# wuliwei9278/primalCR

Measured on NVIDIA B200. Metric: sec_per_outer_iter_primalcrpp_k100_netflix_shape, lower is better.
Workload: dtype f64

## Files before the change

primalcr_b200/csrc/common.cuh:

```cuda
#pragma once
#include <cuda_runtime.h>
#include <stdint.h>
#include <stdio.h>
#include <stdlib.h>
#include <string>
#include <vector>
#include <map>
#include <stdexcept>

namespace pcr {

typedef long long i64;

struct Error : public std::runtime_error {
    int code;
    Error(int c, const std::string &w) : std::runtime_error(w), code(c) {}
};

#define PCR_CUDA(call)                                                                         \
    do {                                                                                       \
        cudaError_t _e = (call);                                                               \
        if (_e != cudaSuccess) {                                                               \
            char _b[512];                                                                      \
            snprintf(_b, sizeof(_b), "CUDA error %s at %s:%d: %s", cudaGetErrorName(_e),       \
// ... 48 lines not shown
                if (tf) {
                    float t0 = 0;
                    cudaEventElapsedTime(&t0, pending.front().a, r.a);
                    fprintf(tf, "%.4f %.4f %s\n", t0, ms, acc[r.id].name.c_str());
                }
            }
            pool.push_back(r.a); pool.push_back(r.b);
        }
        pending.clear();
        if (tf) { fprintf(tf, "# batch end\n"); fclose(tf); }
    }
    void reset() { resolve(); for (auto &a : acc) { a.ms = 0; a.launches = 0; a.bytes = 0; } }
    ~Profiler() { for (auto &r : pending) { cudaEventDestroy(r.a); cudaEventDestroy(r.b); } for (auto e : pool) cudaEventDestroy(e); }
};

struct DevPool {
    std::vector<void *> ptrs;
    i64 bytes = 0;
    cudaStream_t stream = nullptr;
    bool async = false;
    void init(cudaStream_t s) {
        stream = s;
        int dev = 0; cudaMemPool_t mp;
        if (cudaGetDevice(&dev) != cudaSuccess || cudaDeviceGetDefaultMemPool(&mp, dev) != cudaSuccess) { cudaGetLastError(); return; }
        async = true;
        unsigned long long keep = ~0ull;
        cudaMemPoolSetAttribute(mp, cudaMemPoolAttrReleaseThreshold, &keep);
    }
    void *raw_alloc(size_t b) {
        void *p = nullptr;
        if (b == 0) b = 1;
        if (async) PCR_CUDA(cudaMallocAsync(&p, b, stream)); else PCR_CUDA(cudaMalloc(&p, b));
        return p;
    }
    void raw_free(void *p) {
        if (!p) return;
        if (async) cudaFreeAsync(p, stream); else cudaFree(p);
    }
    template <typename T> T *alloc(size_t n) {
        const size_t b = (n > 0 ? n : 1) * sizeof(T);
        void *p = raw_alloc(b);
        ptrs.push_back(p); bytes += (i64)b;
        return (T *)p;
    }
    void release() {
        for (void *p : ptrs) raw_free(p);
        if (async && stream && !ptrs.empty()) cudaStreamSynchronize(stream);
        ptrs.clear(); bytes = 0;
    }
    ~DevPool() { release(); }
};

struct TileList { int32_t *first = nullptr, *nusers = nullptr, *ne = nullptr; i64 *e0 = nullptr; i64 n = 0, nnz = 0; };

struct DevCsr {
    i64 d1 = 0, nnz = 0;
    i64 *row_ptr = nullptr;
    int32_t *item = nullptr;
    int32_t *user = nullptr;
    double *rating = nullptr;
    uint8_t *level = nullptr;
    std::vector<i64> h_row_ptr;
    int32_t *cls_users[3] = {nullptr, nullptr, nullptr};
    int n_cls[3] = {0, 0, 0};
    i64 *heavy_off = nullptr;
    i64 heavy_total = 0;
    i64 *heavy_begin = nullptr, *heavy_end = nullptr;
    i64 max_len = 0;
    TileList tiles[3];
    int32_t *pt_user = nullptr; int32_t *pt_j0 = nullptr; i64 n_pt = 0;
    i64 *pt_ptr = nullptr;
    int32_t *un_seg = nullptr; i64 *un_start = nullptr; i64 n_units = 0;
    i64 *seg_unit_ptr = nullptr;
};

struct SortedMeta {
    double *s = nullptr;
    int32_t *pos = nullptr;
    uint8_t *lev = nullptr;
    int32_t *ub = nullptr, *lb = nullptr;
    int32_t *cnt_lo = nullptr, *cnt_hi = nullptr;
    double *lm_s = nullptr;
    unsigned long long *lm_w0 = nullptr, *lm_w1 = nullptr, *lm_w2 = nullptr;
    uint16_t *ulev = nullptr;
    i64 nnz = 0;
};

static const int HEAVY_CHUNK = 2048;
struct HeavyLM {
    int n_users = 0, n_chunks = 0;
    const int32_t *users = nullptr;
    const i64 *begin = nullptr, *end = nullptr;
    const i64 *off = nullptr;
    const int32_t *chunk_user = nullptr;
    const int32_t *chunk_lo = nullptr;
    const int32_t *chunk0 = nullptr;
    int32_t *ccnt = nullptr;
    int32_t *B = nullptr;
    int32_t *idx = nullptr;
    int32_t *pos = nullptr, *lo = nullptr, *hi = nullptr;
    uint8_t *lev = nullptr;
    double *G = nullptr, *G2 = nullptr;
    double *csum = nullptr;
    i64 htot = 0;
};

struct HeavySortPlan {
    int n_users = 0, n_chunks = 0, max_passes = 0;
    const i64 *begin = nullptr, *end = nullptr;
    const i64 *off = nullptr;
    const int32_t *chunk_user = nullptr;
    const int32_t *chunk_lo = nullptr;
    double *tmp_s = nullptr; int32_t *tmp_pos = nullptr;
};

static const int TILE_CAP = 1024;
static const int TILE_MAX_USERS = 128;
static const int TILE_CAP_M = 2048;
static const int TILE_CAP_L = 4096;
static const int S_CAP = 1024;
static const int L_CAP = 4096;
#ifndef PCR_ROWSUM_CHUNK
#define PCR_ROWSUM_CHUNK 256
#endif
static const int ROWSUM_CHUNK = PCR_ROWSUM_CHUNK;
static const int PAIR_TJ = 256;
static const int MAX_LEVELS = 256;

}
```

primalcr_b200/csrc/engine.cu:

```cuda
#include "kernels.h"
#include "../../include/primalcr.h"
#include "../host/loader.hpp"
#include "../host/textio.hpp"

#include <algorithm>
#include <chrono>
#include <cmath>
#include <cstring>
#include <dlfcn.h>
#include <random>
#include <mutex>

typedef struct { char internal[128]; } pcr_ncclUniqueId;
typedef void *pcr_ncclComm_t;
enum { PCR_NCCL_FLOAT64 = 8, PCR_NCCL_SUM = 0 };

namespace pcr {

struct NcclApi {
    void *h = nullptr;
    int (*GetUniqueId)(pcr_ncclUniqueId *) = nullptr;
    int (*CommInitRank)(pcr_ncclComm_t *, int, pcr_ncclUniqueId, int) = nullptr;
    int (*AllReduce)(const void *, void *, size_t, int, int, pcr_ncclComm_t, cudaStream_t) = nullptr;
    int (*ReduceScatter)(const void *, void *, size_t, int, int, pcr_ncclComm_t, cudaStream_t) = nullptr;
// ... 310 lines not shown
                c0.push_back((int32_t)cu.size());
                for (i64 lo = 0; lo < he[q] - hb[q]; lo += HEAVY_CHUNK) { cu.push_back((int32_t)q); clo.push_back((int32_t)lo); }
            }
            c0.push_back((int32_t)cu.size());
            hv.n_users = (int)cls[2].size(); hv.n_chunks = (int)cu.size(); hv.htot = htot;
            hv.users = X.cls_users[2]; hv.begin = X.heavy_begin; hv.end = X.heavy_end;
            hv.off = upload_vec(hoff_h); hv.chunk_user = upload_vec(cu); hv.chunk_lo = upload_vec(clo); hv.chunk0 = upload_vec(c0);
            hv.ccnt = pool.alloc<int32_t>((size_t)hv.n_chunks * 8); hv.B = pool.alloc<int32_t>((size_t)hv.n_users * 9);
            hv.idx = pool.alloc<int32_t>((size_t)std::max(T - 1, 1) * (size_t)htot);
            hv.G = pool.alloc<double>((size_t)htot); hv.G2 = pool.alloc<double>((size_t)htot);
            hv.pos = pool.alloc<int32_t>((size_t)htot); hv.lo = pool.alloc<int32_t>((size_t)htot); hv.hi = pool.alloc<int32_t>((size_t)htot);
            hv.lev = pool.alloc<uint8_t>((size_t)htot);
            hv.csum = pool.alloc<double>((size_t)hv.n_chunks * 2);
            sync();
        } else {
            alloc_heavy_cta_scratch();
        }
        {
            std::vector<int32_t> useg; std::vector<i64> ustart, supt;
            make_units(X.h_row_ptr, useg, ustart, supt);
            X.n_units = (i64)useg.size();
            X.un_seg = upload_vec(useg); X.un_start = upload_vec(ustart); X.seg_unit_ptr = upload_vec(supt);
            sync();
        }
        lap("classes, tiles, user units");
        col_ptr = pool.alloc<i64>((size_t)d2 + 1);
        csc2csr = pool.alloc<int32_t>((size_t)nnz); csc_user = pool.alloc<int32_t>((size_t)nnz);
        k_build_csc(ctx, pool, X.item, X.user, nnz, d2, col_ptr, csc2csr, csc_user);
        std::vector<i64> h_col((size_t)d2 + 1);
        PCR_CUDA(cudaMemcpyAsync(h_col.data(), col_ptr, sizeof(i64) * ((size_t)d2 + 1), cudaMemcpyDeviceToHost, stream));
        sync();
        PCR_REQUIRE(h_col[d2] == nnz, "item id out of range [0, d2)");
        lap("CSC build (device)");
        {
            const double blk_bytes = getenv("PRIMALCR_UBLOCK_MB") ? atof(getenv("PRIMALCR_UBLOCK_MB")) * 1e6 : 24e6;
            const double u_bytes = (double)d1 * ld * 8.0;
            int nb = (int)std::ceil(u_bytes / blk_bytes);
            if (getenv("PRIMALCR_UBLOCK_MB") == nullptr) {
                const i64 nb_max = std::max<i64>(1, nnz / (32 * std::max<i64>(d2, 1)));
                if (nb > nb_max) nb = (int)nb_max;
            }
            if (nb < 1) nb = 1;
            if (nb > 64) nb = 64;
            const i64 bu = (d1 + nb - 1) / nb > 0 ? (d1 + nb - 1) / nb : 1;
            n_user_blocks = nb;
            std::vector<i64> bpos((size_t)d2 * (nb + 1));
            i64 *bpos_d = nullptr;
            bpos_d = (i64 *)pool.raw_alloc(sizeof(i64) * bpos.size());
            k_csc_block_bounds(ctx, col_ptr, csc_user, d2, nb, bu, bpos_d);
            PCR_CUDA(cudaMemcpyAsync(bpos.data(), bpos_d, sizeof(i64) * bpos.size(), cudaMemcpyDeviceToHost, stream));
            sync();
            pool.raw_free(bpos_d);
            std::vector<int32_t> cseg, cidx; std::vector<i64> cstart, cend, csup((size_t)d2 + 1, 0);
            for (int blk = 0; blk < nb; ++blk)
                for (i64 pcol = 0; pcol < d2; ++pcol) {
                    const i64 lo = bpos[(size_t)pcol * (nb + 1) + blk], hi = blk + 1 == nb ? h_col[pcol + 1] : bpos[(size_t)pcol * (nb + 1) + blk + 1];
                    const i64 collen = h_col[pcol + 1] - h_col[pcol];
                    const i64 chunk = std::max<i64>(ROWSUM_CHUNK, (collen + 47) / 48);
                    for (i64 bb = lo; bb < hi; bb += chunk) {
                        cseg.push_back((int32_t)pcol); cstart.push_back(bb); cend.push_back(std::min(bb + chunk, hi));
                        csup[pcol + 1] += 1;
                    }
                }
            n_cunits = (i64)cseg.size();
            for (i64 pcol = 0; pcol < d2; ++pcol) csup[pcol + 1] += csup[pcol];
            cidx.resize(cseg.size());
            std::vector<i64> fill(csup.begin(), csup.end() - 1);
            for (size_t uu = 0; uu < cseg.size(); ++uu) cidx[fill[cseg[uu]]++] = (int32_t)uu;
            cu_seg = upload_vec(cseg); cu_start = upload_vec(cstart); cu_end = upload_vec(cend);
            col_unit_ptr = upload_vec(csup); col_unit_idx = upload_vec(cidx);
            sync();
        }
        lap("item units (user blocks)");
        m = pool.alloc<double>((size_t)nnz); b = pool.alloc<double>((size_t)nnz); cbuf = pool.alloc<double>((size_t)nnz);
        meta.s = pool.alloc<double>((size_t)nnz); meta.pos = pool.alloc<int32_t>((size_t)nnz);
        meta.lev = pool.alloc<uint8_t>((size_t)nnz);
        meta.ub = pool.alloc<int32_t>((size_t)nnz); meta.lb = pool.alloc<int32_t>((size_t)nnz);
        meta.cnt_lo = pool.alloc<int32_t>((size_t)nnz); meta.cnt_hi = pool.alloc<int32_t>((size_t)nnz);
        meta.nnz = nnz;
        if (use_tiles) {
            meta.lm_s = pool.alloc<double>((size_t)nnz);
            meta.lm_w0 = pool.alloc<unsigned long long>((size_t)nnz); meta.lm_w1 = pool.alloc<unsigned long long>((size_t)nnz);
            if (T > 5) meta.lm_w2 = pool.alloc<unsigned long long>((size_t)nnz);
            meta.ulev = pool.alloc<uint16_t>((size_t)d1 * 8);
            PCR_CUDA(cudaMemsetAsync(meta.ulev, 0, sizeof(uint16_t) * (size_t)d1 * 8, stream));
        }
        const size_t vn = (size_t)d2 * ld, un = (size_t)d1 * ld;
        U = pool.alloc<double>(un);
        d2p = world > 1 ? (d2 + world - 1) / world * world : d2;
        vs_rows = d2p / std::max(world, 1); vs_row0 = (i64)rank * vs_rows;
        sharded_cg = world > 1 && (double)vn * 8.0 >= 64e6;
        if (const char *sc_env = getenv("PRIMALCR_SHARDED_CG")) sharded_cg = world > 1 && atoi(sc_env) != 0;
        const size_t vnp = (size_t)d2p * ld;
        g = pool.alloc<double>(vnp); delta = pool.alloc<double>(vnp); rr = pool.alloc<double>(vnp);
        p = pool.alloc<double>(vnp); Hp = pool.alloc<double>(vnp); V = pool.alloc<double>(vnp); Vnew = pool.alloc<double>(vnp);
        for (double *vec : {g, delta, rr, p, Hp, V, Vnew}) PCR_CUDA(cudaMemsetAsync(vec, 0, sizeof(double) * vnp, stream));
        partial = pool.alloc<double>((size_t)std::max(X.n_units, n_cunits) * ld);
        us.g = pool.alloc<double>(un); us.delta = pool.alloc<double>(un); us.rr = pool.alloc<double>(un);
        us.p = pool.alloc<double>(un); us.Hp = pool.alloc<double>(un); us.Unew = pool.alloc<double>(un);
        us.err = pool.alloc<double>((size_t)d1); us.step = pool.alloc<double>((size_t)d1);
        us.prev_obj = pool.alloc<double>((size_t)d1); us.obj_new = pool.alloc<double>((size_t)d1);
        us.loss = pool.alloc<double>((size_t)d1);
        us.cg_active = pool.alloc<uint8_t>((size_t)d1); us.ls_active = pool.alloc<uint8_t>((size_t)d1);
        us.skipped = pool.alloc<uint8_t>((size_t)d1);
        us.cg_its = pool.alloc<int32_t>((size_t)d1); us.ls_trials = pool.alloc<int32_t>((size_t)d1);
        k_fill(ctx, us.loss, d1, 0.0);
        has_pairs = pool.alloc<uint8_t>((size_t)d1);
        k_has_pairs(ctx, X, has_pairs);
        obj_item = pool.alloc<double>((size_t)X.n_pt);
        ensure_eval_buffers(X);
        sync();
        lap("work buffers");
        has_train = true;
    }

    void alloc_heavy_cta_scratch() {
        if (h_v != nullptr || X.heavy_total <= 0) return;
        const size_t htot = (size_t)X.heavy_total;
        h_v = pool.alloc<double>(htot); h_p1 = pool.alloc<double>(htot);
        h_p2 = pool.alloc<double>(htot); h_acc = pool.alloc<double>(htot);
        h_cnt = pool.alloc<int32_t>(htot);
    }
    void ensure_heavy_windows() {
        if (!heavy_chunked || heavy_windows_valid || X.n_cls[2] == 0) return;
        alloc_heavy_cta_scratch();
        k_windows(ctx, 2, X.cls_users[2], X.n_cls[2], nullptr, X.row_ptr, meta, T, X.heavy_off, h_cnt);
        heavy_windows_valid = true;
    }
    i64 ev_cap_pt = 0, ev_cap_d1 = 0, ev_cap_nnz = 0;
    void ensure_eval_buffers(const DevCsr &C) {
        if (C.n_pt > ev_cap_pt) { ev_err_item = pool.alloc<i64>((size_t)C.n_pt); ev_cap_pt = C.n_pt; }
        if (C.d1 > ev_cap_d1 || ev_a == nullptr) {
            ev_err_user = pool.alloc<i64>((size_t)C.d1);
            ev_a = pool.alloc<double>((size_t)C.d1); ev_b = pool.alloc<double>((size_t)C.d1);
            ev_c = pool.alloc<double>((size_t)C.d1); ev_d = pool.alloc<double>((size_t)C.d1); ev_cap_d1 = C.d1;
        }
    }

    void set_test(i64 nnz, const i64 *row_ptr, const int32_t *item, const double *rating) {
        bind();
        PCR_REQUIRE(has_train, "load the training set first");
        PCR_REQUIRE(!has_test, "test set already loaded");
        build_csr_common(XT, d1, nnz, row_ptr, item, rating);
        ev_score_t = pool.alloc<double>((size_t)nnz);
        ensure_eval_buffers(XT);
        has_test = nnz > 0;
    }

    void put_matrix(const double *h, i64 rows, double *dst) {
        if (rows == 0) return;
        if (ld == k) {
            PCR_CUDA(cudaMemcpyAsync(dst, h, sizeof(double) * (size_t)rows * k, cudaMemcpyHostToDevice, stream));
        } else {
            double *tmp = (double *)pool.raw_alloc(sizeof(double) * (size_t)rows * k);
            PCR_CUDA(cudaMemcpyAsync(tmp, h, sizeof(double) * (size_t)rows * k, cudaMemcpyHostToDevice, stream));
            k_pad_copy(ctx, tmp, rows, k, ld, dst);
            PCR_CUDA(cudaStreamSynchronize(stream));
            pool.raw_free(tmp);
        }
    }
    void get_matrix(const double *src, i64 rows, double *h) {
        if (rows == 0) return;
        if (ld == k) {
            PCR_CUDA(cudaMemcpyAsync(h, src, sizeof(double) * (size_t)rows * k, cudaMemcpyDeviceToHost, stream));
        } else {
            PCR_CUDA(cudaMemcpy2DAsync(h, sizeof(double) * k, src, sizeof(double) * ld, sizeof(double) * k, (size_t)rows,
                                       cudaMemcpyDeviceToHost, stream));
        }
// ... 797 lines not shown
```

primalcr_b200/csrc/k_tiles.cu:

```cuda
#include "kernels.h"
#include <math_constants.h>

namespace pcr {

#define FULL 0xffffffffu
#define LAUNCH(ctx, name, bytes, kernel, grid, block, smem, ...)                         \
    do {                                                                                 \
        (ctx).prof->begin(name, (ctx).stream, (double)(bytes));                          \
        kernel<<<(grid), (block), (smem), (ctx).stream>>>(__VA_ARGS__);                  \
        (ctx).prof->end((ctx).stream);                                                   \
        PCR_CUDA(cudaGetLastError());                                                    \
    } while (0)

static const int TE = 4;

template <int CAP>
struct TileShared {
    int ustart[TILE_MAX_USERS + 1];
    uint8_t uact[TILE_MAX_USERS];
    uint8_t ul[CAP];
};

template <typename VT, int TT, int TH, typename ValF, typename LevF>
__device__ __forceinline__ void tile_level_scan(const TileShared<TH * TE> &ts, int ne, int T, VT *S, VT *wagg ,
                                                int *wflag , ValF val, LevF lev) {
    constexpr int SLOTS = TH * TE + TILE_MAX_USERS;
    const int tid = threadIdx.x, lane = tid & 31, warp = tid >> 5;
    const int lo = tid * TE;
    VT agg[TT];
#pragma unroll
    for (int t = 0; t < TT; ++t) agg[t] = (VT)0;
    int flag = 0;
#pragma unroll
    for (int q = 0; q < TE; ++q) {
        const int i = lo + q;
        if (i < ne) {
            const int u = ts.ul[i];
            if (i == ts.ustart[u]) {
#pragma unroll
                for (int t = 0; t < TT; ++t) agg[t] = (VT)0;
                flag = 1;
            }
            const int l = lev(i);
            const VT v = val(i);
#pragma unroll
            for (int t = 0; t < TT; ++t) agg[t] += (t == l) ? v : (VT)0;
        }
    }
    VT inc[TT];
#pragma unroll
    for (int t = 0; t < TT; ++t) inc[t] = agg[t];
    int finc = flag;
#pragma unroll
    for (int o = 1; o < 32; o <<= 1) {
        const int of = __shfl_up_sync(FULL, finc, o);
#pragma unroll
        for (int t = 0; t < TT; ++t) {
            const VT ov = __shfl_up_sync(FULL, inc[t], o);
            if (lane >= o && !finc) inc[t] += ov;
        }
        if (lane >= o) finc |= of;
    }
    if (lane == 31) {
#pragma unroll
        for (int t = 0; t < TT; ++t) wagg[warp * TT + t] = inc[t];
        wflag[warp] = finc;
    }
    VT exc[TT];
    int fexc = __shfl_up_sync(FULL, finc, 1);
#pragma unroll
    for (int t = 0; t < TT; ++t) { exc[t] = __shfl_up_sync(FULL, inc[t], 1); if (lane == 0) exc[t] = (VT)0; }
    if (lane == 0) fexc = 0;
    __syncthreads();
    VT carry[TT];
#pragma unroll
    for (int t = 0; t < TT; ++t) carry[t] = (VT)0;
    for (int w = 0; w < warp; ++w) {
        const int wf = wflag[w];
#pragma unroll
        for (int t = 0; t < TT; ++t) carry[t] = wf ? wagg[w * TT + t] : carry[t] + wagg[w * TT + t];
    }
#pragma unroll
    for (int t = 0; t < TT; ++t) carry[t] = fexc ? exc[t] : carry[t] + exc[t];
#pragma unroll
    for (int q = 0; q < TE; ++q) {
        const int i = lo + q;
        if (i < ne) {
            const int u = ts.ul[i];
            if (i == ts.ustart[u]) {
#pragma unroll
                for (int t = 0; t < TT; ++t) carry[t] = (VT)0;
            }
            const int slot = i + u;
#pragma unroll
            for (int t = 0; t < TT; ++t) if (t < T) S[t * SLOTS + slot] = carry[t];
            const int l = lev(i);
            const VT v = val(i);
#pragma unroll
            for (int t = 0; t < TT; ++t) carry[t] += (t == l) ? v : (VT)0;
            if (i + 1 == ts.ustart[u + 1]) {
#pragma unroll
                for (int t = 0; t < TT; ++t) if (t < T) S[t * SLOTS + slot + 1] = carry[t];
            }
        }
    }
    __syncthreads();
}

template <int TH>
__device__ __forceinline__ bool tile_users(TileShared<TH * TE> &ts, int first_user, int n_users, i64 e0,
                                           const i64 *__restrict__ row_ptr, const uint8_t *__restrict__ active) {
    const int tid = threadIdx.x;
    int any = 0;
    for (int u = tid; u <= n_users; u += TH) {
        const i64 rp = row_ptr[first_user + u];
        ts.ustart[u] = (int)(rp - e0);
        if (u < n_users) {
            const uint8_t a = active ? active[first_user + u] : (uint8_t)1;
            ts.uact[u] = a;
            if (a && row_ptr[first_user + u + 1] > rp) any = 1;
        }
    }
    return __syncthreads_or(any) != 0;
}

#ifndef PCR_PREP_MINB
#define PCR_PREP_MINB 4
#endif
template <int TT, int TH>
__global__ void __launch_bounds__(TH, TH == 256 ? PCR_PREP_MINB : (TH == 512 ? 2 : 1)) tile_prepare_kernel(const int32_t *__restrict__ tile_first,
                                                          const int32_t *__restrict__ tile_nusers,
                                                          const i64 *__restrict__ tile_e0, const int32_t *__restrict__ tile_ne,
                                                          const uint8_t *__restrict__ active,
                                                          const i64 *__restrict__ row_ptr, const int32_t *__restrict__ user_of,
                                                          const double *__restrict__ m, const uint8_t *__restrict__ level,
                                                          double *__restrict__ s_out, int32_t *__restrict__ pos_out,
                                                          uint8_t *__restrict__ lev_out, int32_t *__restrict__ ub_out,
                                                          int32_t *__restrict__ lb_out, int32_t *__restrict__ lo_out,
                                                          int32_t *__restrict__ hi_out, int T, SortedMeta lm) {
    constexpr int CAP = TH * TE, SLOTS = CAP + TILE_MAX_USERS;
    extern __shared__ __align__(16) unsigned char smraw[];
    __shared__ TileShared<CAP> ts;
    __shared__ int wagg[TH / 32 * TT];
    __shared__ int wflag[TH / 32];
    double *keys = reinterpret_cast<double *>(smraw);
    unsigned long long *pk = reinterpret_cast<unsigned long long *>(keys + CAP);
    int *C = reinterpret_cast<int *>(pk + CAP);
    uint32_t *tag = reinterpret_cast<uint32_t *>(C + T * SLOTS);
    uint8_t *slev = reinterpret_cast<uint8_t *>(tag + CAP);
    uint8_t *lev0 = slev + CAP;
    __shared__ int s_fallback;
    const int tid = threadIdx.x;
    const int first_user = tile_first[blockIdx.x], n_users = tile_nusers[blockIdx.x];
    const i64 e0 = tile_e0[blockIdx.x];
    const int ne = tile_ne[blockIdx.x];
    bool users_done = false;
    if (active) {
        if (!tile_users<TH>(ts, first_user, n_users, e0, row_ptr, active)) return;
        users_done = true;
    }
    int np2 = 1;
    while (np2 < ne) np2 <<= 1;
    double r_m[TE]; int r_u[TE]; uint8_t r_l[TE];
#pragma unroll
    for (int q = 0; q < TE; ++q) {
        const int i = tid + q * TH;
        r_m[q] = CUDART_INF; r_u[q] = 0xFFFF; r_l[q] = 0;
        if (i < ne) { r_m[q] = m[e0 + i]; r_u[q] = user_of[e0 + i] - first_user; r_l[q] = level[e0 + i]; }
    }
    if (!users_done) tile_users<TH>(ts, first_user, n_users, e0, row_ptr, active);
#pragma unroll
    for (int q = 0; q < TE; ++q) {
        const int i = tid + q * TH;
        if (i < np2) {
            keys[i] = r_m[q];
            if (i < ne) {
                const float f = (float)r_m[q] + 0.0f;
                const uint32_t b = __float_as_uint(f);
                const uint32_t fk = b ^ ((b >> 31) ? 0xFFFFFFFFu : 0x80000000u);
                pk[i] = ((unsigned long long)r_u[q] << 45) | ((unsigned long long)fk << 13) | (unsigned long long)i;
                ts.ul[i] = (uint8_t)r_u[q]; lev0[i] = r_l[q];
            } else {
                pk[i] = ~0ull;
            }
        }
    }
    if (tid == 0) s_fallback = 0;
    __syncthreads();
    {
        const int p0 = tid * TE;
        const bool live = ((tid & ~31) * TE) < np2;
        unsigned long long ek[TE];
#pragma unroll
        for (int q = 0; q < TE; ++q) ek[q] = pk[p0 + q];
        for (int k = 2; k <= np2; k <<= 1) {
            for (int j = k >> 1; j >= 32 * TE; j >>= 1) {
                __syncthreads();
#pragma unroll
                for (int q = 0; q < TE; ++q) pk[p0 + q] = ek[q];
                __syncthreads();
                const int m = j / TE;
                const int pp = (tid ^ m) * TE;
                const bool keep_min = (((tid & m) == 0) == ((p0 & k) == 0));
#pragma unroll
                for (int q = 0; q < TE; ++q) {
                    const unsigned long long o = pk[pp + q];
// ... 17 lines not shown
                    for (int q = 0; q < 2; ++q) {
                        const unsigned long long a = ek[q], b = ek[q + 2];
                        if ((a > b) == asc) { ek[q] = b; ek[q + 2] = a; }
                    }
                }
#pragma unroll
                for (int q = 0; q < TE; q += 2) {
                    const bool asc = (((p0 + q) & k) == 0);
                    const unsigned long long a = ek[q], b = ek[q + 1];
                    if ((a > b) == asc) { ek[q] = b; ek[q + 1] = a; }
                }
            }
        }
        __syncthreads();
#pragma unroll
        for (int q = 0; q < TE; ++q) pk[p0 + q] = ek[q];
        __syncthreads();
    }
    {
        int round = 0;
        for (;;) {
            int swapped = 0;
            for (int phase = 0; phase < 2; ++phase) {
                for (int i = 2 * tid + phase; i + 1 < ne; i += 2 * TH) {
                    const unsigned long long a = pk[i], b = pk[i + 1];
                    if ((a >> 13) == (b >> 13)) {
                        const int ia = (int)(a & 0x1FFFu), ib = (int)(b & 0x1FFFu);
                        const double ka = keys[ia], kb = keys[ib];
                        if (ka > kb || (ka == kb && ia > ib)) { pk[i] = b; pk[i + 1] = a; swapped = 1; }
                    }
                }
                __syncthreads();
            }
            if (!__syncthreads_or(swapped)) break;
            if (++round >= 48) { if (tid == 0) s_fallback = 1; break; }
        }
        __syncthreads();
    }
    const bool fallback = s_fallback != 0;
    double srt[TE];
#pragma unroll
    for (int q = 0; q < TE; ++q) {
        const int i = tid + q * TH;
        srt[q] = CUDART_INF;
        if (i < ne && !fallback) srt[q] = keys[(int)(pk[i] & 0x1FFFu)];
    }
    __syncthreads();
#pragma unroll
    for (int q = 0; q < TE; ++q) {
        const int i = tid + q * TH;
        if (i < np2) {
            if (!fallback) {
                if (i < ne) { keys[i] = srt[q]; tag[i] = ((uint32_t)ts.ul[i] << 16) | (uint32_t)(pk[i] & 0x1FFFu); }
            } else {
                keys[i] = r_m[q];
                tag[i] = i < ne ? (((uint32_t)r_u[q] << 16) | (uint32_t)i) : 0xFFFFFFFFu;
            }
        }
    }
    __syncthreads();
    if (fallback) {
        for (int k = 2; k <= np2; k <<= 1) {
            for (int j = k >> 1; j > 0; j >>= 1) {
                for (int t = tid; t < (np2 >> 1); t += TH) {
                    const int i = ((t & ~(j - 1)) << 1) | (t & (j - 1));
                    const int p = i | j;
                    const bool asc = (i & k) == 0;
                    const uint32_t ti = tag[i], tp = tag[p];
                    const double ki = keys[i], kp = keys[p];
                    const bool gt = ((ti >> 16) != (tp >> 16)) ? (ti > tp) : ((ki > kp) || (ki == kp && ti > tp));
                    if (gt == asc) { keys[i] = kp; keys[p] = ki; tag[i] = tp; tag[p] = ti; }
                }
                __syncthreads();
            }
        }
    }
    for (int i = tid; i < ne; i += TH) {
        const int src = (int)(tag[i] & 0xFFFFu);
        const uint8_t l = lev0[src];
        slev[i] = l;
        if (ts.uact[ts.ul[i]]) { s_out[e0 + i] = keys[i]; pos_out[e0 + i] = (int32_t)(e0 + src); lev_out[e0 + i] = l; }
    }
    __syncthreads();
    tile_level_scan<int, TT, TH>(ts, ne, T, C, wagg, wflag, [](int) { return 1; }, [&](int i) { return (int)slev[i]; });
    for (int i = tid; i < ne; i += TH) {
        const int u = ts.ul[i];
        if (!ts.uact[u]) continue;
        const int u0 = ts.ustart[u], n = ts.ustart[u + 1] - u0, x = i - u0;
        const double *kk = keys + u0;
        const double sj = kk[x];
        const double hi = __dadd_rn(sj, 1.0), lo = __dadd_rn(sj, -1.0);
        int a = x + 1, b = n;
        while (a < b) { const int mid = (a + b) >> 1; if (kk[mid] <= hi) a = mid + 1; else b = mid; }
        const int ub = a;
        a = 0; b = x;
        while (a < b) { const int mid = (a + b) >> 1; if (kk[mid] < lo) a = mid + 1; else b = mid; }
        const int lb = a;
        const int base = u0 + u, l = slev[i];
        int chi = 0, clo = 0;
        for (int t = 0; t < T; ++t) {
            const int *Ct = C + t * SLOTS + base;
            if (t > l) chi += Ct[ub];
            else if (t < l) clo += Ct[n] - Ct[lb];
        }
        ub_out[e0 + i] = ub; lb_out[e0 + i] = lb; lo_out[e0 + i] = clo; hi_out[e0 + i] = chi;
        int run = 0, r = 0;
        uint16_t other[TT];
#pragma unroll
        for (int t = 0; t < TT; ++t) {
            other[t] = 0;
            if (t < T) {
                const int *Ct = C + t * SLOTS + base;
                if (t == l) r = run + Ct[x];
                else other[t] = (uint16_t)(run + (t > l ? Ct[ub] : Ct[lb]));
                run += Ct[n];
            }
        }
        const i64 gi = e0 + u0 + r;
        unsigned long long w1 = 0ull, w2 = 0ull;
#pragma unroll
        for (int t = 0; t < TT; ++t) {
            if (t < T && t != l) {
                const int slot = t < l ? t : t - 1;
                if (slot < 4) w1 |= (unsigned long long)other[t] << (13 * slot);
                else          w2 |= (unsigned long long)other[t] << (13 * (slot - 4));
            }
        }
        lm.lm_s[gi] = sj;
        lm.lm_w0[gi] = (unsigned long long)(tag[i] & 0xFFFFu) | ((unsigned long long)clo << 13) | ((unsigned long long)chi << 26) |
                       ((unsigned long long)l << 39) | ((unsigned long long)u << 42);
        lm.lm_w1[gi] = w1;
        if (TT > 5) lm.lm_w2[gi] = w2;
    }
    for (int w = tid; w < n_users * T; w += TH) {
        const int u = w / T, t = w - u * T;
        const int n = ts.ustart[u + 1] - ts.ustart[u];
        if (ts.uact[u]) lm.ulev[(i64)(first_user + u) * 8 + t] = (uint16_t)(n > 0 ? C[t * SLOTS + ts.ustart[u] + u + n] : 0);
    }
}

#ifndef PCR_LM_MINB
#define PCR_LM_MINB 5
#endif
template <int MODE, int TT, int TH>
__global__ void __launch_bounds__(TH, TH == 256 ? PCR_LM_MINB : (TH == 512 ? 2 : 1)) tile_lm_sweep_kernel(const int32_t *__restrict__ tile_first,
                                                           const int32_t *__restrict__ tile_nusers,
                                                           const i64 *__restrict__ tile_e0, const int32_t *__restrict__ tile_ne,
                                                           const uint8_t *__restrict__ active,
                                                           const i64 *__restrict__ row_ptr, const int32_t *__restrict__ user_of,
                                                           SortedMeta lm, const double *__restrict__ b_g,
                                                           double *__restrict__ c_out, double *__restrict__ obj_user, int T) {
    constexpr int CAP = TH * TE, SLOTS = CAP + TILE_MAX_USERS;
    __shared__ TileShared<CAP> ts;
    __shared__ double wagg[TH / 32];
    __shared__ int wflag[TH / 32];
    extern __shared__ __align__(16) unsigned char smraw[];
    double *G = reinterpret_cast<double *>(smraw);
    double *sval = G + SLOTS;
    double *G2 = sval + CAP;
    double *stg = sval + CAP;
    __shared__ double Kt[TILE_MAX_USERS * TT], Kt2[MODE == 2 ? TILE_MAX_USERS * TT : 1];
    __shared__ uint16_t Bt[TILE_MAX_USERS * (TT + 1)];
    const int tid = threadIdx.x;
    const int first_user = tile_first[blockIdx.x], n_users = tile_nusers[blockIdx.x];
    const i64 e0 = tile_e0[blockIdx.x];
    const int ne = tile_ne[blockIdx.x];
    bool users_done = false;
    if (active) {
        if (!tile_users<TH>(ts, first_user, n_users, e0, row_ptr, active)) return;
        users_done = true;
    }
    unsigned long long r_w0[TE], r_w1[TE], r_w2[TT > 5 ? TE : 1];
    double r_v[TE];
#pragma unroll
    for (int q = 0; q < TE; ++q) {
        const int i = tid + q * TH;
        r_w0[q] = 0ull; r_w1[q] = 0ull; r_v[q] = 0.0;
        if (TT > 5) r_w2[q] = 0ull;
        if (i < ne) {
            r_w0[q] = lm.lm_w0[e0 + i];
            r_w1[q] = lm.lm_w1[e0 + i];
            if (TT > 5) r_w2[q] = lm.lm_w2[e0 + i];
            if (MODE != 1) r_v[q] = lm.lm_s[e0 + i];
        }
    }
    if (MODE == 1) {
#pragma unroll
        for (int q = 0; q < TE; ++q) { const int i = tid + q * TH; if (i < ne) stg[i] = b_g[e0 + i]; }
    }
    if (!users_done) tile_users<TH>(ts, first_user, n_users, e0, row_ptr, active);
    for (int u = tid; u < n_users; u += TH) {
        int run = 0;
        for (int t = 0; t < T; ++t) { Bt[u * (TT + 1) + t] = (uint16_t)run; run += lm.ulev[(i64)(first_user + u) * 8 + t]; }
        Bt[u * (TT + 1) + T] = (uint16_t)run;
    }
#pragma unroll
    for (int q = 0; q < TE; ++q) {
        const int i = tid + q * TH;
        if (i < ne) { ts.ul[i] = (uint8_t)((r_w0[q] >> 42) & 0x7Full); if (MODE != 1) sval[i] = MODE == 2 ? r_v[q] - 1.0 : r_v[q]; }
    }
    __syncthreads();
    if (MODE == 1) {
#pragma unroll
        for (int q = 0; q < TE; ++q) {
            const int i = tid + q * TH;
            if (i < ne) { r_v[q] = stg[(int)(r_w0[q] & 0x1FFFull)]; sval[i] = r_v[q]; }
        }
        __syncthreads();
    }
    tile_level_scan<double, 1, TH>(ts, ne, 1, G, wagg, wflag, [&](int i) { return sval[i]; }, [](int) { return 0; });
    if (MODE == 2)
        tile_level_scan<double, 1, TH>(ts, ne, 1, G2, wagg, wflag, [&](int i) { const double d = sval[i]; return d * d; }, [](int) { return 0; });
    for (int w = tid; w < n_users * T; w += TH) {
        const int u = w / T, l = w - u * T;
        const int base = ts.ustart[u] + u;
        const uint16_t *B = Bt + u * (TT + 1);
        double k1 = 0.0, k2 = 0.0;
        for (int t = 0; t < T; ++t) {
            if (t > l) { k1 -= G[base + B[t]]; if (MODE == 2) k2 -= G2[base + B[t]]; }
            else if (t < l && MODE != 2) k1 += G[base + B[t + 1]];
        }
        Kt[u * TT + l] = k1;
        if (MODE == 2) Kt2[u * TT + l] = k2;
    }
    __syncthreads();
    double objj[TE];
#pragma unroll
    for (int q = 0; q < TE; ++q) {
        const int i = tid + q * TH;
        objj[q] = 0.0;
        if (i >= ne) continue;
        const unsigned long long w0 = r_w0[q];
        const int u = (int)((w0 >> 42) & 0x7Full);
        if (!ts.uact[u]) continue;
        const int base = ts.ustart[u] + u, l = (int)((w0 >> 39) & 7ull);
        double acc = Kt[u * TT + l], acc2 = MODE == 2 ? Kt2[u * TT + l] : 0.0;
#pragma unroll
        for (int t = 0; t < TT - 1; ++t) {
            if (t < T - 1) {
                const unsigned long long wi = (TT > 5 && t >= 4) ? r_w2[TT > 5 ? q : 0] >> (13 * (t - 4)) : r_w1[q] >> (13 * t);
                const int at = base + (int)(wi & 0x1FFFull);
                if (t >= l) { acc += G[at]; if (MODE == 2) acc2 += G2[at]; }
                else if (MODE != 2) acc -= G[at];
            }
        }
        const double v = r_v[q];
        const double hi = (double)(int)((w0 >> 26) & 0x1FFFull);
        if (MODE == 2) {
            objj[q] = hi * (v * v) - 2.0 * v * acc + acc2;
        } else {
            const double lo = (double)(int)((w0 >> 13) & 0x1FFFull);
            const double cc = MODE == 0 ? lo * (v - 1.0) + hi * (v + 1.0) - acc : (lo + hi) * v - acc;
            if (active == nullptr) stg[(int)(w0 & 0x1FFFull)] = 2.0 * cc;
            else c_out[e0 + (i64)(w0 & 0x1FFFull)] = 2.0 * cc;
        }
    }
    if (MODE != 2 && active == nullptr) {
        __syncthreads();
        for (int i = tid; i < ne; i += TH) c_out[e0 + i] = stg[i];
    }
    if (MODE == 2) {
        __syncthreads();
#pragma unroll
        for (int q = 0; q < TE; ++q) { const int i = tid + q * TH; if (i < ne) sval[i] = objj[q]; }
        __syncthreads();
        tile_level_scan<double, 1, TH>(ts, ne, 1, G, wagg, wflag, [&](int i) { return sval[i]; }, [](int) { return 0; });
        for (int u = tid; u < n_users; u += TH) {
            const int n = ts.ustart[u + 1] - ts.ustart[u];
            if (n > 0 && ts.uact[u]) obj_user[first_user + u] = G[ts.ustart[u] + u + n];
        }
    }
}

static size_t prepare_smem(int T, int cap) { return (size_t)cap * 16 + (size_t)T * (cap + TILE_MAX_USERS) * 4 + (size_t)cap * 4 + 2 * (size_t)cap; }

template <typename K>
static void set_smem(K kernel, size_t bytes) {
    PCR_CUDA(cudaFuncSetAttribute(kernel, cudaFuncAttributeMaxDynamicSharedMemorySize, (int)bytes));
}

void k_tile_prepare(Ctx &c, const DevCsr &X, int geo, const uint8_t *active, const double *m, SortedMeta &meta, int T) {
    const TileList &L = X.tiles[geo];
    if (L.n <= 0) return;
    PCR_REQUIRE(T <= 8, "tile kernels support at most 8 rating levels");
    const double bytes = (double)L.nnz * (13 + 29 + 24);
#define PREP_ARGS L.first, L.nusers, L.e0, L.ne, active, X.row_ptr, X.user, m, X.level, meta.s, meta.pos, meta.lev, meta.ub, meta.lb, meta.cnt_lo, meta.cnt_hi, T, meta
#define PREP_LAUNCH(TT, TH, NAME) { const size_t sm = prepare_smem(T, TH * TE); set_smem(tile_prepare_kernel<TT, TH>, sm); \
        LAUNCH(c, NAME, bytes, (tile_prepare_kernel<TT, TH>), (unsigned)L.n, TH, sm, PREP_ARGS); }
    if (geo == 0)      { if (T <= 5) PREP_LAUNCH(5, 256, "tile_prepare") else PREP_LAUNCH(8, 256, "tile_prepare") }
    else if (geo == 1) { PCR_REQUIRE(T <= 5, "medium tiles need T <= 5"); PREP_LAUNCH(5, 512, "tile_prepare_M") }
    else               { PCR_REQUIRE(T <= 5, "large tiles need T <= 5"); PREP_LAUNCH(5, 1024, "tile_prepare_L") }
#undef PREP_LAUNCH
#undef PREP_ARGS
}

void k_tile_sweep(Ctx &c, int mode, const DevCsr &X, int geo, const uint8_t *active, const SortedMeta &meta, const double *b,
                  double *c_out, double *obj_user, int T) {
    const TileList &L = X.tiles[geo];
    if (L.n <= 0) return;
    PCR_REQUIRE(T <= 8, "tile kernels support at most 8 rating levels");
    const double per = mode == 2 ? (16 + 8) : (16 + 8 + 8);
    const double bytes = (double)L.nnz * per;
    const unsigned grid = (unsigned)L.n;
#define LM_ARGS L.first, L.nusers, L.e0, L.ne, active, X.row_ptr, X.user, meta, b, c_out, obj_user, T
#define LM_LAUNCH(MODE, TT, TH, NAME) { const size_t sm = ((size_t)(TH * TE + TILE_MAX_USERS) * (MODE == 2 ? 2 : 1) + TH * TE * (MODE == 2 ? 1 : 2)) * 8; \
    set_smem(tile_lm_sweep_kernel<MODE, TT, TH>, sm); LAUNCH(c, NAME, bytes, (tile_lm_sweep_kernel<MODE, TT, TH>), grid, TH, sm, LM_ARGS); }
#define LM_MODE(MODE, NAME)                                                                                         \
    if (geo == 0)      { if (T <= 5) { LM_LAUNCH(MODE, 5, 256, NAME) } else { LM_LAUNCH(MODE, 8, 256, NAME) } }   \
    else if (geo == 1) { LM_LAUNCH(MODE, 5, 512, NAME "_M") }                                                    \
    else               { LM_LAUNCH(MODE, 5, 1024, NAME "_L") }
    if (mode == 0) { LM_MODE(0, "lm_sweep_grad") }
    else if (mode == 1) { LM_MODE(1, "lm_sweep_hv") }
    else { LM_MODE(2, "lm_sweep_obj") }
#undef LM_MODE
#undef LM_LAUNCH
#undef LM_ARGS
}

}
```

Baseline: 0.2559.

## Restructure tile LM sweep scans to fuse G/G2 and trim shared memory

Measured after the change: 0.2562 (median of 6 runs). About the same (+0.1%).

```diff
diff --git a/primalcr_b200/csrc/common.cuh b/primalcr_b200/csrc/common.cuh
--- a/primalcr_b200/csrc/common.cuh
+++ b/primalcr_b200/csrc/common.cuh
@@ -154,7 +154,7 @@
     int32_t *cnt_lo = nullptr, *cnt_hi = nullptr;
     double *lm_s = nullptr;
     unsigned long long *lm_w0 = nullptr, *lm_w1 = nullptr, *lm_w2 = nullptr;
-    uint16_t *ulev = nullptr;
+    uint16_t *ublk = nullptr;
     i64 nnz = 0;
 };
 
diff --git a/primalcr_b200/csrc/engine.cu b/primalcr_b200/csrc/engine.cu
--- a/primalcr_b200/csrc/engine.cu
+++ b/primalcr_b200/csrc/engine.cu
@@ -416,8 +416,8 @@
             meta.lm_s = pool.alloc<double>((size_t)nnz);
             meta.lm_w0 = pool.alloc<unsigned long long>((size_t)nnz); meta.lm_w1 = pool.alloc<unsigned long long>((size_t)nnz);
             if (T > 5) meta.lm_w2 = pool.alloc<unsigned long long>((size_t)nnz);
-            meta.ulev = pool.alloc<uint16_t>((size_t)d1 * 8);
-            PCR_CUDA(cudaMemsetAsync(meta.ulev, 0, sizeof(uint16_t) * (size_t)d1 * 8, stream));
+            meta.ublk = pool.alloc<uint16_t>((size_t)d1 * 8);
+            PCR_CUDA(cudaMemsetAsync(meta.ublk, 0, sizeof(uint16_t) * (size_t)d1 * 8, stream));
         }
         const size_t vn = (size_t)d2 * ld, un = (size_t)d1 * ld;
         U = pool.alloc<double>(un);
diff --git a/primalcr_b200/csrc/k_tiles.cu b/primalcr_b200/csrc/k_tiles.cu
--- a/primalcr_b200/csrc/k_tiles.cu
+++ b/primalcr_b200/csrc/k_tiles.cu
@@ -21,15 +21,17 @@
     uint8_t ul[CAP];
 };
 
-template <typename VT, int TT, int TH, typename ValF, typename LevF>
-__device__ __forceinline__ void tile_level_scan(const TileShared<TH * TE> &ts, int ne, int T, VT *S, VT *wagg ,
-                                                int *wflag , ValF val, LevF lev) {
-    constexpr int SLOTS = TH * TE + TILE_MAX_USERS;
+template <typename VT, int NS>
+struct ScanLane { VT exc[NS]; int fexc; };
+
+template <typename VT, int NS, int TH, typename ValF>
+__device__ __forceinline__ ScanLane<VT, NS> tile_scan_warp(const TileShared<TH * TE> &ts, int ne, VT *wagg ,
+                                                         int *wflag , ValF vals) {
     const int tid = threadIdx.x, lane = tid & 31, warp = tid >> 5;
     const int lo = tid * TE;
-    VT agg[TT];
-#pragma unroll
-    for (int t = 0; t < TT; ++t) agg[t] = (VT)0;
+    VT agg[NS];
+#pragma unroll
+    for (int s = 0; s < NS; ++s) agg[s] = (VT)0;
     int flag = 0;
 #pragma unroll
     for (int q = 0; q < TE; ++q) {
@@ -38,50 +40,56 @@
             const int u = ts.ul[i];
             if (i == ts.ustart[u]) {
 #pragma unroll
-                for (int t = 0; t < TT; ++t) agg[t] = (VT)0;
+                for (int s = 0; s < NS; ++s) agg[s] = (VT)0;
                 flag = 1;
             }
-            const int l = lev(i);
-            const VT v = val(i);
-#pragma unroll
-            for (int t = 0; t < TT; ++t) agg[t] += (t == l) ? v : (VT)0;
-        }
-    }
-    VT inc[TT];
-#pragma unroll
-    for (int t = 0; t < TT; ++t) inc[t] = agg[t];
+            VT v[NS];
+            vals(i, v);
+#pragma unroll
+            for (int s = 0; s < NS; ++s) agg[s] += v[s];
+        }
+    }
+    VT inc[NS];
+#pragma unroll
+    for (int s = 0; s < NS; ++s) inc[s] = agg[s];
     int finc = flag;
 #pragma unroll
     for (int o = 1; o < 32; o <<= 1) {
         const int of = __shfl_up_sync(FULL, finc, o);
 #pragma unroll
-        for (int t = 0; t < TT; ++t) {
-            const VT ov = __shfl_up_sync(FULL, inc[t], o);
-            if (lane >= o && !finc) inc[t] += ov;
+        for (int s = 0; s < NS; ++s) {
+            const VT ov = __shfl_up_sync(FULL, inc[s], o);
+            if (lane >= o && !finc) inc[s] += ov;
         }
         if (lane >= o) finc |= of;
     }
     if (lane == 31) {
 #pragma unroll
-        for (int t = 0; t < TT; ++t) wagg[warp * TT + t] = inc[t];
+        for (int s = 0; s < NS; ++s) wagg[warp * NS + s] = inc[s];
         wflag[warp] = finc;
     }
-    VT exc[TT];
-    int fexc = __shfl_up_sync(FULL, finc, 1);
-#pragma unroll
-    for (int t = 0; t < TT; ++t) { exc[t] = __shfl_up_sync(FULL, inc[t], 1); if (lane == 0) exc[t] = (VT)0; }
-    if (lane == 0) fexc = 0;
-    __syncthreads();
-    VT carry[TT];
-#pragma unroll
-    for (int t = 0; t < TT; ++t) carry[t] = (VT)0;
+    ScanLane<VT, NS> r;
+    r.fexc = __shfl_up_sync(FULL, finc, 1);
+    if (lane == 0) r.fexc = 0;
+#pragma unroll
+    for (int s = 0; s < NS; ++s) { r.exc[s] = __shfl_up_sync(FULL, inc[s], 1); if (lane == 0) r.exc[s] = (VT)0; }
+    return r;
+}
+
+template <typename VT, int NS, int TH, typename ValF, typename ExclF, typename TotF>
+__device__ __forceinline__ void tile_scan_emit(const TileShared<TH * TE> &ts, int ne, const VT *wagg, const int *wflag,
+                                               const ScanLane<VT, NS> &r, ValF vals, ExclF excl, TotF total) {
+    const int warp = threadIdx.x >> 5, lo = threadIdx.x * TE;
+    VT carry[NS];
+#pragma unroll
+    for (int s = 0; s < NS; ++s) carry[s] = (VT)0;
     for (int w = 0; w < warp; ++w) {
         const int wf = wflag[w];
 #pragma unroll
-        for (int t = 0; t < TT; ++t) carry[t] = wf ? wagg[w * TT + t] : carry[t] + wagg[w * TT + t];
-    }
-#pragma unroll
-    for (int t = 0; t < TT; ++t) carry[t] = fexc ? exc[t] : carry[t] + exc[t];
+        for (int s = 0; s < NS; ++s) carry[s] = wf ? wagg[w * NS + s] : carry[s] + wagg[w * NS + s];
+    }
+#pragma unroll
+    for (int s = 0; s < NS; ++s) carry[s] = r.fexc ? r.exc[s] : carry[s] + r.exc[s];
 #pragma unroll
     for (int q = 0; q < TE; ++q) {
         const int i = lo + q;
@@ -89,30 +97,24 @@
             const int u = ts.ul[i];
             if (i == ts.ustart[u]) {
 #pragma unroll
-                for (int t = 0; t < TT; ++t) carry[t] = (VT)0;
+                for (int s = 0; s < NS; ++s) carry[s] = (VT)0;
             }
             const int slot = i + u;
-#pragma unroll
-            for (int t = 0; t < TT; ++t) if (t < T) S[t * SLOTS + slot] = carry[t];
-            const int l = lev(i);
-            const VT v = val(i);
-#pragma unroll
-            for (int t = 0; t < TT; ++t) carry[t] += (t == l) ? v : (VT)0;
-            if (i + 1 == ts.ustart[u + 1]) {
-#pragma unroll
-                for (int t = 0; t < TT; ++t) if (t < T) S[t * SLOTS + slot + 1] = carry[t];
-            }
-        }
-    }
-    __syncthreads();
+            excl(slot, carry);
+            VT v[NS];
+            vals(i, v);
+#pragma unroll
+            for (int s = 0; s < NS; ++s) carry[s] += v[s];
+            if (i + 1 == ts.ustart[u + 1]) total(u, slot + 1, carry);
+        }
+    }
 }
 
 template <int TH>
-__device__ __forceinline__ bool tile_users(TileShared<TH * TE> &ts, int first_user, int n_users, i64 e0,
-                                           const i64 *__restrict__ row_ptr, const uint8_t *__restrict__ active) {
-    const int tid = threadIdx.x;
+__device__ __forceinline__ int tile_users_stage(TileShared<TH * TE> &ts, int first_user, int n_users, i64 e0,
+                                                const i64 *__restrict__ row_ptr, const uint8_t *__restrict__ active) {
     int any = 0;
-    for (int u = tid; u <= n_users; u += TH) {
+    for (int u = threadIdx.x; u <= n_users; u += TH) {
         const i64 rp = row_ptr[first_user + u];
         ts.ustart[u] = (int)(rp - e0);
         if (u < n_users) {
@@ -121,7 +123,13 @@
             if (a && row_ptr[first_user + u + 1] > rp) any = 1;
         }
     }
-    return __syncthreads_or(any) != 0;
+    return any;
+}
+
+template <int TH>
+__device__ __forceinline__ bool tile_users(TileShared<TH * TE> &ts, int first_user, int n_users, i64 e0,
+                                           const i64 *__restrict__ row_ptr, const uint8_t *__restrict__ active) {
+    return __syncthreads_or(tile_users_stage<TH>(ts, first_user, n_users, e0, row_ptr, active)) != 0;
 }
 
 #ifndef PCR_PREP_MINB
@@ -305,7 +313,21 @@
         if (ts.uact[ts.ul[i]]) { s_out[e0 + i] = keys[i]; pos_out[e0 + i] = (int32_t)(e0 + src); lev_out[e0 + i] = l; }
     }
     __syncthreads();
-    tile_level_scan<int, TT, TH>(ts, ne, T, C, wagg, wflag, [](int) { return 1; }, [&](int i) { return (int)slev[i]; });
+    {
+        auto one = [&](int i, int *v) {
+            const int l = slev[i];
+#pragma unroll
+            for (int t = 0; t < TT; ++t) v[t] = t == l ? 1 : 0;
+        };
+        auto put = [&](int slot, const int *c) {
+#pragma unroll
+            for (int t = 0; t < TT; ++t) if (t < T) C[t * SLOTS + slot] = c[t];
+        };
+        const ScanLane<int, TT> r = tile_scan_warp<int, TT, TH>(ts, ne, wagg, wflag, one);
+        __syncthreads();
+        tile_scan_emit<int, TT, TH>(ts, ne, wagg, wflag, r, one, put, [&](int, int slot, const int *c) { put(slot, c); });
+        __syncthreads();
+    }
     for (int i = tid; i < ne; i += TH) {
         const int u = ts.ul[i];
         if (!ts.uact[u]) continue;
@@ -355,15 +377,22 @@
         lm.lm_w1[gi] = w1;
         if (TT > 5) lm.lm_w2[gi] = w2;
     }
-    for (int w = tid; w < n_users * T; w += TH) {
-        const int u = w / T, t = w - u * T;
+    for (int u = tid; u < n_users; u += TH) {
+        if (!ts.uact[u]) continue;
         const int n = ts.ustart[u + 1] - ts.ustart[u];
-        if (ts.uact[u]) lm.ulev[(i64)(first_user + u) * 8 + t] = (uint16_t)(n > 0 ? C[t * SLOTS + ts.ustart[u] + u + n] : 0);
+        union { uint4 v; uint16_t h[8]; } bt;
+        int run = 0;
+#pragma unroll
+        for (int t = 0; t < 8; ++t) {
+            bt.h[t] = (uint16_t)run;
+            if (t < T && n > 0) run += C[t * SLOTS + ts.ustart[u] + u + n];
+        }
+        reinterpret_cast<uint4 *>(lm.ublk)[first_user + u] = bt.v;
     }
 }
 
 #ifndef PCR_LM_MINB
-#define PCR_LM_MINB 5
+#define PCR_LM_MINB 6
 #endif
 template <int MODE, int TT, int TH>
 __global__ void __launch_bounds__(TH, TH == 256 ? PCR_LM_MINB : (TH == 512 ? 2 : 1)) tile_lm_sweep_kernel(const int32_t *__restrict__ tile_first,
@@ -374,70 +403,61 @@
                                                            SortedMeta lm, const double *__restrict__ b_g,
                                                            double *__restrict__ c_out, double *__restrict__ obj_user, int T) {
     constexpr int CAP = TH * TE, SLOTS = CAP + TILE_MAX_USERS;
+    constexpr int NS = MODE == 2 ? 2 : 1;
     __shared__ TileShared<CAP> ts;
-    __shared__ double wagg[TH / 32];
+    __shared__ double wagg[TH / 32 * NS];
     __shared__ int wflag[TH / 32];
+    __shared__ uint16_t spos[MODE == 1 ? CAP : 1];
+    __shared__ uint4 sbt[TILE_MAX_USERS];
+    __shared__ double Kt[TILE_MAX_USERS * TT], Kt2[MODE == 2 ? TILE_MAX_USERS * TT : 1];
     extern __shared__ __align__(16) unsigned char smraw[];
     double *G = reinterpret_cast<double *>(smraw);
-    double *sval = G + SLOTS;
-    double *G2 = sval + CAP;
-    double *stg = sval + CAP;
-    __shared__ double Kt[TILE_MAX_USERS * TT], Kt2[MODE == 2 ? TILE_MAX_USERS * TT : 1];
-    __shared__ uint16_t Bt[TILE_MAX_USERS * (TT + 1)];
+    double *G2 = G + SLOTS;
+    double *stg = G + NS * SLOTS;
     const int tid = threadIdx.x;
     const int first_user = tile_first[blockIdx.x], n_users = tile_nusers[blockIdx.x];
     const i64 e0 = tile_e0[blockIdx.x];
     const int ne = tile_ne[blockIdx.x];
-    bool users_done = false;
-    if (active) {
-        if (!tile_users<TH>(ts, first_user, n_users, e0, row_ptr, active)) return;
-        users_done = true;
-    }
-    unsigned long long r_w0[TE], r_w1[TE], r_w2[TT > 5 ? TE : 1];
-    double r_v[TE];
-#pragma unroll
-    for (int q = 0; q < TE; ++q) {
-        const int i = tid + q * TH;
-        r_w0[q] = 0ull; r_w1[q] = 0ull; r_v[q] = 0.0;
-        if (TT > 5) r_w2[q] = 0ull;
+    if (active && !tile_users<TH>(ts, first_user, n_users, e0, row_ptr, active)) return;
+    unsigned long long r_w0[TE];
+#pragma unroll
+    for (int q = 0; q < TE; ++q) {
+        const int i = tid + q * TH;
+        r_w0[q] = 0ull;
         if (i < ne) {
             r_w0[q] = lm.lm_w0[e0 + i];
-            r_w1[q] = lm.lm_w1[e0 + i];
-            if (TT > 5) r_w2[q] = lm.lm_w2[e0 + i];
-            if (MODE != 1) r_v[q] = lm.lm_s[e0 + i];
-        }
-    }
-    if (MODE == 1) {
-#pragma unroll
-        for (int q = 0; q < TE; ++q) { const int i = tid + q * TH; if (i < ne) stg[i] = b_g[e0 + i]; }
-    }
-    if (!users_done) tile_users<TH>(ts, first_user, n_users, e0, row_ptr, active);
-    for (int u = tid; u < n_users; u += TH) {
-        int run = 0;
-        for (int t = 0; t < T; ++t) { Bt[u * (TT + 1) + t] = (uint16_t)run; run += lm.ulev[(i64)(first_user + u) * 8 + t]; }
-        Bt[u * (TT + 1) + T] = (uint16_t)run;
-    }
-#pragma unroll
-    for (int q = 0; q < TE; ++q) {
-        const int i = tid + q * TH;
-        if (i < ne) { ts.ul[i] = (uint8_t)((r_w0[q] >> 42) & 0x7Full); if (MODE != 1) sval[i] = MODE == 2 ? r_v[q] - 1.0 : r_v[q]; }
+            if (MODE == 1) stg[i] = b_g[e0 + i];
+            else stg[i] = MODE == 2 ? lm.lm_s[e0 + i] - 1.0 : lm.lm_s[e0 + i];
+        }
+    }
+    if (!active) tile_users_stage<TH>(ts, first_user, n_users, e0, row_ptr, active);
+    for (int u = tid; u < n_users; u += TH) sbt[u] = reinterpret_cast<const uint4 *>(lm.ublk)[first_user + u];
+#pragma unroll
+    for (int q = 0; q < TE; ++q) {
+        const int i = tid + q * TH;
+        if (i < ne) {
+            ts.ul[i] = (uint8_t)((r_w0[q] >> 42) & 0x7Full);
+            if (MODE == 1) spos[i] = (uint16_t)(r_w0[q] & 0x1FFFull);
+        }
     }
     __syncthreads();
-    if (MODE == 1) {
-#pragma unroll
-        for (int q = 0; q < TE; ++q) {
-            const int i = tid + q * TH;
-            if (i < ne) { r_v[q] = stg[(int)(r_w0[q] & 0x1FFFull)]; sval[i] = r_v[q]; }
-        }
-        __syncthreads();
-    }
-    tile_level_scan<double, 1, TH>(ts, ne, 1, G, wagg, wflag, [&](int i) { return sval[i]; }, [](int) { return 0; });
-    if (MODE == 2)
-        tile_level_scan<double, 1, TH>(ts, ne, 1, G2, wagg, wflag, [&](int i) { const double d = sval[i]; return d * d; }, [](int) { return 0; });
+    {
+        auto stream = [&](int i, double *v) {
+            const double d = MODE == 1 ? stg[spos[i]] : stg[i];
+            v[0] = d;
+            if (MODE == 2) v[NS - 1] = d * d;
+        };
+        auto put = [&](int slot, const double *c) { G[slot] = c[0]; if (MODE == 2) G2[slot] = c[NS - 1]; };
+        const ScanLane<double, NS> r = tile_scan_warp<double, NS, TH>(ts, ne, wagg, wflag, stream);
+        __syncthreads();
+        tile_scan_emit<double, NS, TH>(ts, ne, wagg, wflag, r, stream, put, [&](int, int slot, const double *c) { put(slot, c); });
+        __syncthreads();
+    }
     for (int w = tid; w < n_users * T; w += TH) {
         const int u = w / T, l = w - u * T;
+        if (!ts.uact[u]) continue;
         const int base = ts.ustart[u] + u;
-        const uint16_t *B = Bt + u * (TT + 1);
+        const uint16_t *B = reinterpret_cast<const uint16_t *>(&sbt[u]);
         double k1 = 0.0, k2 = 0.0;
         for (int t = 0; t < T; ++t) {
             if (t > l) { k1 -= G[base + B[t]]; if (MODE == 2) k2 -= G2[base + B[t]]; }
@@ -447,11 +467,22 @@
         if (MODE == 2) Kt2[u * TT + l] = k2;
     }
     __syncthreads();
-    double objj[TE];
-#pragma unroll
-    for (int q = 0; q < TE; ++q) {
-        const int i = tid + q * TH;
-        objj[q] = 0.0;
+    unsigned long long r_w1[TE], r_w2[TT > 5 ? TE : 1];
+    double r_v[MODE == 1 ? 1 : TE];
+#pragma unroll
+    for (int q = 0; q < TE; ++q) {
+        const int i = tid + q * TH;
+        if (i < ne) {
+            r_w1[q] = lm.lm_w1[e0 + i];
+            if (TT > 5) r_w2[q] = lm.lm_w2[e0 + i];
+            if (MODE != 1) r_v[q] = lm.lm_s[e0 + i];
+        }
+    }
+    double objj[MODE == 2 ? TE : 1];
+#pragma unroll
+    for (int q = 0; q < TE; ++q) {
+        const int i = tid + q * TH;
+        if (MODE == 2) objj[q] = 0.0;
         if (i >= ne) continue;
         const unsigned long long w0 = r_w0[q];
         const int u = (int)((w0 >> 42) & 0x7Full);
@@ -467,15 +498,16 @@
                 else if (MODE != 2) acc -= G[at];
             }
         }
-        const double v = r_v[q];
+        const int pos = (int)(w0 & 0x1FFFull);
+        const double v = MODE == 1 ? stg[pos] : r_v[MODE == 1 ? 0 : q];
         const double hi = (double)(int)((w0 >> 26) & 0x1FFFull);
         if (MODE == 2) {
             objj[q] = hi * (v * v) - 2.0 * v * acc + acc2;
         } else {
             const double lo = (double)(int)((w0 >> 13) & 0x1FFFull);
             const double cc = MODE == 0 ? lo * (v - 1.0) + hi * (v + 1.0) - acc : (lo + hi) * v - acc;
-            if (active == nullptr) stg[(int)(w0 & 0x1FFFull)] = 2.0 * cc;
-            else c_out[e0 + (i64)(w0 & 0x1FFFull)] = 2.0 * cc;
+            if (active == nullptr) stg[pos] = 2.0 * cc;
+            else c_out[e0 + pos] = 2.0 * cc;
         }
     }
     if (MODE != 2 && active == nullptr) {
@@ -483,15 +515,14 @@
         for (int i = tid; i < ne; i += TH) c_out[e0 + i] = stg[i];
     }
     if (MODE == 2) {
-        __syncthreads();
-#pragma unroll
-        for (int q = 0; q < TE; ++q) { const int i = tid + q * TH; if (i < ne) sval[i] = objj[q]; }
-        __syncthreads();
-        tile_level_scan<double, 1, TH>(ts, ne, 1, G, wagg, wflag, [&](int i) { return sval[i]; }, [](int) { return 0; });
-        for (int u = tid; u < n_users; u += TH) {
-            const int n = ts.ustart[u + 1] - ts.ustart[u];
-            if (n > 0 && ts.uact[u]) obj_user[first_user + u] = G[ts.ustart[u] + u + n];
-        }
+#pragma unroll
+        for (int q = 0; q < TE; ++q) { const int i = tid + q * TH; if (i < ne) stg[i] = objj[q]; }
+        __syncthreads();
+        auto term = [&](int i, double *v) { v[0] = stg[i]; };
+        const ScanLane<double, 1> r = tile_scan_warp<double, 1, TH>(ts, ne, wagg, wflag, term);
+        __syncthreads();
+        tile_scan_emit<double, 1, TH>(ts, ne, wagg, wflag, r, term, [](int, const double *) {},
+                                      [&](int u, int, const double *c) { if (ts.uact[u]) obj_user[first_user + u] = c[0]; });
     }
 }
 
@@ -526,7 +557,7 @@
     const double bytes = (double)L.nnz * per;
     const unsigned grid = (unsigned)L.n;
 #define LM_ARGS L.first, L.nusers, L.e0, L.ne, active, X.row_ptr, X.user, meta, b, c_out, obj_user, T
-#define LM_LAUNCH(MODE, TT, TH, NAME) { const size_t sm = ((size_t)(TH * TE + TILE_MAX_USERS) * (MODE == 2 ? 2 : 1) + TH * TE * (MODE == 2 ? 1 : 2)) * 8; \
+#define LM_LAUNCH(MODE, TT, TH, NAME) { const size_t sm = ((size_t)(TH * TE + TILE_MAX_USERS) * (MODE == 2 ? 2 : 1) + TH * TE) * 8; \
     set_smem(tile_lm_sweep_kernel<MODE, TT, TH>, sm); LAUNCH(c, NAME, bytes, (tile_lm_sweep_kernel<MODE, TT, TH>), grid, TH, sm, LM_ARGS); }
 #define LM_MODE(MODE, NAME)                                                                                         \
     if (geo == 0)      { if (T <= 5) { LM_LAUNCH(MODE, 5, 256, NAME) } else { LM_LAUNCH(MODE, 8, 256, NAME) } }   \
```
